# merlresearch/tssep

Hardware: AMD Instinct MI355X
Metric: frames/sec fwd+bwd, 4-spk TS-SEP, 16kHz 4s chunks (higher is better)
Workload: dtype bf16x3+f32

## Files before the change

tssep_amd/csrc/feat.hip:

```cpp
#include <math.h>
#include "common.h"

namespace {

__device__ __forceinline__ unsigned ord(float f) {
  const unsigned u = __float_as_uint(f);
  return (u & 0x80000000u) ? ~u : (u | 0x80000000u);
}
__device__ __forceinline__ float unord(unsigned u) {
  return __uint_as_float((u & 0x80000000u) ? (u & 0x7fffffffu) : ~u);
}

constexpr int MAXF = 1032;
constexpr int GSLOTS = 64;

struct FeatWs {
  unsigned* gmax;
  unsigned* umax;
  int* range;
  float* fbT;
  float* db;
};
constexpr int STAT_TF = 0, STAT_T = 1, STAT_F = 2;
__host__ __device__ inline int64_t feat_nmax(int64_t B, int F, int stat) { return stat == STAT_T ? B * F : B; }
__host__ __device__ inline FeatWs feat_ws(void* ws, int64_t B , int n_mels) {
  FeatWs w;
  char* p = (char*)ws;
  w.gmax = (unsigned*)p;
  w.umax = (unsigned*)(p + GSLOTS * 4);
  const int64_t off1 = GSLOTS * 4 + ((B * 4 + 15) / 16) * 16;
  w.range = (int*)(p + off1);
  const int64_t off2 = off1 + (((int64_t)2 * n_mels * 4 + 15) / 16) * 16;
  w.fbT = (float*)(p + off2);
  w.db = (float*)(p + off2 + (int64_t)n_mels * MAXF * 4);
  return w;
}

__global__ __launch_bounds__(64) void feat_init_kernel(void* ws, int64_t B, const float* __restrict__ fb,
                                                       int F, int n_mels) {
  FeatWs w = feat_ws(ws, B, n_mels);
  const int lane = threadIdx.x, m = blockIdx.x;
  if (m == 0) w.gmax[lane] = 0u;
  for (int64_t b = (int64_t)m * 64 + lane; b < B; b += (int64_t)gridDim.x * 64) w.umax[b] = 0u;
  if (m >= n_mels) return;
  float lo = (float)F, hi = 0.f;
  for (int f = lane; f < F; f += 64) {
    const float v = fb[(int64_t)f * n_mels + m];
    w.fbT[(int64_t)m * MAXF + f] = v;
    if (v != 0.f) { lo = fminf(lo, (float)f); hi = fmaxf(hi, (float)(f + 1)); }
  }
  lo = -wave_max(-lo);
  hi = wave_max(hi);
  if (lane == 0) {
    w.range[2 * m] = hi == 0.f ? 0 : (int)lo;
    w.range[2 * m + 1] = (int)hi;
  }
}

constexpr int FPW = 4;
constexpr int CWMAX = 2 * MAXF;
constexpr int LMELS = 128;

__global__ __launch_bounds__(256) void feat_pass1_kernel(const float2* __restrict__ X, int64_t B,
                                                         int64_t T, int F,
                                                         const float* __restrict__ fb, int n_mels,
                                                         int n_mfcc, void* ws, int stat, int log_mels) {
  __shared__ float pw[4][MAXF];
  __shared__ float cw[CWMAX];
  __shared__ int clo[LMELS], chi[LMELS], coff[LMELS + 1];
  __shared__ int s_packed;
  FeatWs w = feat_ws(ws, feat_nmax(B, F, stat), n_mels);
  const int tid = threadIdx.x, lane = tid & 63, wave = tid >> 6;
  if (n_mfcc > 0) {
    if (tid < n_mels && tid < LMELS) {
      clo[tid] = w.range[2 * tid];
      chi[tid] = w.range[2 * tid + 1];
    }
    __syncthreads();
    if (tid == 0) {
      int tot = 0;
      const int nm = n_mels < LMELS ? n_mels : LMELS;
      for (int m = 0; m < nm; ++m) {
        coff[m] = tot;
        const int wd = chi[m] - clo[m];
        tot += wd > 0 ? wd : 0;
      }
      coff[nm] = tot;
      s_packed = (n_mels <= LMELS && tot <= CWMAX) ? 1 : 0;
    }
    __syncthreads();
    if (s_packed)
      for (int m = wave; m < n_mels; m += 4)
        for (int f = clo[m] + lane; f < chi[m]; f += 64) cw[coff[m] + f - clo[m]] = w.fbT[(int64_t)m * MAXF + f];
    __syncthreads();
  }
  const bool packed = n_mfcc > 0 && s_packed;
  float dbmax = -INFINITY;
  for (int it = 0; it < FPW; ++it) {
    const int64_t frame = ((int64_t)blockIdx.x * FPW + it) * 4 + wave;
    if (frame >= B * T) break;
    const float2* x = X + frame * F;
    float amax = 0.f;
    float2 xv[17];
#pragma unroll
    for (int r = 0; r < 17; ++r) {
      const int f = lane + 64 * r;
      xv[r] = f < F ? x[f] : make_float2(0.f, 0.f);
    }
#pragma unroll
    for (int r = 0; r < 17; ++r) {
      const int f = lane + 64 * r;
      if (f < F) {
        const float p = xv[r].x * xv[r].x + xv[r].y * xv[r].y;
        pw[wave][f] = p;
        amax = fmaxf(amax, sqrtf(p));
        if (stat == STAT_T) {
          unsigned* slot = w.umax + (frame / T) * F + f;
          const unsigned o_ = ord(sqrtf(p));
          if (o_ > __hip_atomic_load(slot, __ATOMIC_RELAXED, __HIP_MEMORY_SCOPE_AGENT)) atomicMax(slot, o_);
        }
      }
    }
    __builtin_amdgcn_fence(__ATOMIC_RELEASE, "wavefront");
    __builtin_amdgcn_wave_barrier();
    __builtin_amdgcn_fence(__ATOMIC_ACQUIRE, "wavefront");
    amax = wave_max(amax);
    if (lane == 0 && stat == STAT_TF) atomicMax(w.umax + frame / T, ord(amax));
    if (n_mfcc > 0) {
      for (int m0 = 0; m0 < n_mels; m0 += 64) {
        float mine = 0.f;
        const int mm = n_mels - m0 < 64 ? n_mels - m0 : 64;
        if (lane < mm) {
          const int m = m0 + lane;
          const int lo = packed ? clo[m] : w.range[2 * m], hi = packed ? chi[m] : w.range[2 * m + 1];
          const float* frow = packed ? cw + coff[m] - lo : w.fbT + (int64_t)m * MAXF;
          const float* prow = pw[wave];
          float s0 = 0.f, s1 = 0.f, s2 = 0.f, s3 = 0.f;
          int f = lo;
          for (; f + 3 < hi; f += 4) {
            s0 = fmaf(prow[f], frow[f], s0);
            s1 = fmaf(prow[f + 1], frow[f + 1], s1);
            s2 = fmaf(prow[f + 2], frow[f + 2], s2);
            s3 = fmaf(prow[f + 3], frow[f + 3], s3);
          }
          if (f < hi) s0 = fmaf(prow[f], frow[f], s0);
          if (f + 1 < hi) s1 = fmaf(prow[f + 1], frow[f + 1], s1);
          if (f + 2 < hi) s2 = fmaf(prow[f + 2], frow[f + 2], s2);
          mine = (s0 + s1) + (s2 + s3);
        }
        if (lane < mm) {
          const float db = log_mels ? logf(mine + 1e-6f) : 10.0f * log10f(fmaxf(mine, 1e-10f));
          w.db[frame * n_mels + m0 + lane] = db;
          dbmax = fmaxf(dbmax, db);
        }
      }
    }
    __builtin_amdgcn_fence(__ATOMIC_RELEASE, "wavefront");
    __builtin_amdgcn_wave_barrier();
    __builtin_amdgcn_fence(__ATOMIC_ACQUIRE, "wavefront");
  }
  if (n_mfcc > 0) {
    dbmax = wave_max(dbmax);
    if (lane == 0 && dbmax > -INFINITY) atomicMax(w.gmax + (blockIdx.x & (GSLOTS - 1)), ord(dbmax));
  }
}

__global__ __launch_bounds__(256) void feat_pass2_kernel(const float2* __restrict__ X, int64_t B,
                                                         int64_t T, int F,
                                                         const float* __restrict__ dct, int n_mels,
                                                         int n_mfcc, float top_db,
                                                         float* __restrict__ out, int64_t ld_out,
                                                         const void* ws, int stat) {
  __shared__ float dbl[4][64];
  FeatWs w = feat_ws(const_cast<void*>(ws), feat_nmax(B, F, stat), n_mels);
  const int lane = threadIdx.x & 63, wave = threadIdx.x >> 6;
  const int64_t frame = (int64_t)blockIdx.x * 4 + wave;
  const bool valid = frame < B * T;
  float* o = out + (valid ? frame : 0) * ld_out;
  if (n_mfcc > 0) {
    const float floor_db = top_db < 0.f ? -INFINITY : wave_max(unord(w.gmax[lane])) - top_db;
    for (int m0 = 0; m0 < n_mels; m0 += 64) {
      if (valid && m0 + lane < n_mels)
        dbl[wave][lane] = fmaxf(w.db[frame * n_mels + m0 + lane], floor_db);
      __syncthreads();
      if (valid) {
        const int mm = n_mels - m0 < 64 ? n_mels - m0 : 64;
        for (int c = lane; c < n_mfcc; c += 64) {
          float s = m0 ? o[c] : 0.f;
          for (int m = 0; m < mm; ++m) s = fmaf(dbl[wave][m], dct[(int64_t)(m0 + m) * n_mfcc + c], s);
          o[c] = s;
        }
      }
      __syncthreads();
    }
  }
  if (!valid) return;
  const float2* x = X + frame * F;
  float2 xv[17];
#pragma unroll
  for (int r = 0; r < 17; ++r) {
    const int f = lane + 64 * r;
    xv[r] = f < F ? x[f] : make_float2(0.f, 0.f);
  }
  if (stat == STAT_TF) {
    const float scale = (float)(M_E - 1.0) / unord(w.umax[frame / T]);
#pragma unroll
    for (int r = 0; r < 17; ++r) {
      const int f = lane + 64 * r;
      if (f < F) o[n_mfcc + f] = log1pf(sqrtf(xv[r].x * xv[r].x + xv[r].y * xv[r].y) * scale);
    }
    return;
  }
  float fmx = 0.f;
  if (stat == STAT_F) {
#pragma unroll
    for (int r = 0; r < 17; ++r)
      if (lane + 64 * r < F) fmx = fmaxf(fmx, sqrtf(xv[r].x * xv[r].x + xv[r].y * xv[r].y));
    fmx = wave_max(fmx);
  }
#pragma unroll
  for (int r = 0; r < 17; ++r) {
    const int f = lane + 64 * r;
    if (f < F) {
      const float norm = stat == STAT_F ? fmx : unord(w.umax[(frame / T) * F + f]);
      o[n_mfcc + f] = log1pf(sqrtf(xv[r].x * xv[r].x + xv[r].y * xv[r].y) * ((float)(M_E - 1.0) / norm));
    }
  }
}

}

extern "C" int64_t tssep_feat_workspace_bytes(int64_t B, int64_t T, int n_mels, int F, int stat_axis) {
  if (stat_axis < 0 || stat_axis > 2 || F <= 0) return 0;
  FeatWs w = feat_ws(nullptr, feat_nmax(B, F, stat_axis), n_mels);
  return (int64_t)((char*)w.db - (char*)nullptr) + B * T * (int64_t)n_mels * 4 + 16;
}

extern "C" int tssep_feat_fwd(const float* X, int64_t B, int64_t T, int F, const float* fb,
                              const float* dct, int n_mels, int n_mfcc, float top_db, int stat_axis,
                              float* out, int64_t ld_out, void* ws, void* stream) {
  if (!X || !out || !ws) return TSSEP_E_NULL;
  if (n_mfcc > 0 && (!fb || !dct)) return TSSEP_E_NULL;
  if (B <= 0 || T <= 0 || F <= 0 || F > MAXF || ld_out < n_mfcc + F) return TSSEP_E_SHAPE;
  if (n_mfcc > 0 && (n_mels <= 0 || n_mels > 1024)) return TSSEP_E_SHAPE;
  if (n_mfcc == 0) n_mels = 0;
  if (stat_axis < 0 || stat_axis > 2) return TSSEP_E_SHAPE;
  if ((((uintptr_t)X) & 7u) || (((uintptr_t)ws) & 15u)) return TSSEP_E_ALIGN;
  hipStream_t s = (hipStream_t)stream;
  const int nm = n_mels > 0 ? n_mels : 1;
  const int64_t nmax = feat_nmax(B, F, stat_axis);
  const int64_t nb0 = (nmax + 64 * 16 - 1) / (64 * 16);
  hipLaunchKernelGGL(feat_init_kernel, dim3((unsigned)(nb0 > nm ? (nb0 > 4096 ? 4096 : nb0) : nm)), dim3(64), 0, s, ws, nmax, fb, F, n_mels);
  const unsigned blocks = (unsigned)((B * T + 3) / 4);
  const unsigned blocks1 = (unsigned)((B * T + 4 * FPW - 1) / (4 * FPW));
  hipLaunchKernelGGL(feat_pass1_kernel, dim3(blocks1), dim3(256), 0, s, (const float2*)X, B, T, F,
                     fb, n_mels, n_mfcc, ws, stat_axis, top_db < 0.f ? 1 : 0);
  hipLaunchKernelGGL(feat_pass2_kernel, dim3(blocks), dim3(256), 0, s, (const float2*)X, B, T, F,
                     dct, n_mels, n_mfcc, top_db, out, ld_out, ws, stat_axis);
  return tssep_launch_status();
}
```

Before: 2.159 million.

## Restructure feature kernels as persistent waves with prefetched buffer loads and LDS DCT

```diff
diff --git a/tssep_amd/csrc/feat.hip b/tssep_amd/csrc/feat.hip
--- a/tssep_amd/csrc/feat.hip
+++ b/tssep_amd/csrc/feat.hip
@@ -1,5 +1,6 @@
 #include <math.h>
 #include "common.h"
+#include "gemm_common.h"
 
 namespace {
 
@@ -57,107 +58,172 @@
   }
 }
 
-constexpr int FPW = 4;
-constexpr int CWMAX = 2 * MAXF;
+typedef __amdgpu_buffer_rsrc_t srd_t;
+typedef unsigned u32x4_t __attribute__((ext_vector_type(4)));
+__device__ __forceinline__ srd_t frame_srd(const float2* X, int64_t frame, int64_t nframes, int F) {
+  const bool in = frame < nframes;
+  return __builtin_amdgcn_make_buffer_rsrc(const_cast<float2*>(X + (in ? frame : 0) * F), 0, in ? F * 8 : 0, 0x00020000);
+}
+__device__ __forceinline__ f32x4 bload4(srd_t r, int voff) {
+  return __builtin_bit_cast(f32x4, __builtin_amdgcn_raw_buffer_load_b128(r, voff, 0, 0));
+}
+#define WAVE_SYNC()                                          \
+  do {                                                       \
+    __builtin_amdgcn_fence(__ATOMIC_RELEASE, "wavefront");   \
+    __builtin_amdgcn_wave_barrier();                         \
+    __builtin_amdgcn_fence(__ATOMIC_ACQUIRE, "wavefront");   \
+  } while (0)
+__device__ __forceinline__ float lane_value(float v, int l) {
+  return __int_as_float(__builtin_amdgcn_readlane(__float_as_int(v), l));
+}
+__device__ __forceinline__ float power(float re, float im) {
+#pragma clang fp contract(off)
+  return re * re + im * im;
+}
+
+constexpr int p1_occ(int NL) { return NL <= 5 ? 6 : 4; }
 constexpr int LMELS = 128;
-
-__global__ __launch_bounds__(256) void feat_pass1_kernel(const float2* __restrict__ X, int64_t B,
-                                                         int64_t T, int F,
-                                                         const float* __restrict__ fb, int n_mels,
-                                                         int n_mfcc, void* ws, int stat, int log_mels) {
-  __shared__ float pw[4][MAXF];
-  __shared__ float cw[CWMAX];
+constexpr int CWMAX = 2 * MAXF + 6 * LMELS;
+
+__host__ __device__ inline int seg_len(int lo, int hi) { return hi > lo ? ((hi + 3) & ~3) - (lo & ~3) : 0; }
+
+__device__ __forceinline__ float band_sum_global(const FeatWs& w, int m, const float* prow) {
+  const int lo = w.range[2 * m], hi = w.range[2 * m + 1];
+  const float* frow = w.fbT + (int64_t)m * MAXF;
+  float s0 = 0.f, s1 = 0.f, s2 = 0.f, s3 = 0.f;
+  int f = lo;
+  for (; f + 3 < hi; f += 4) {
+    s0 = fmaf(prow[f], frow[f], s0);
+    s1 = fmaf(prow[f + 1], frow[f + 1], s1);
+    s2 = fmaf(prow[f + 2], frow[f + 2], s2);
+    s3 = fmaf(prow[f + 3], frow[f + 3], s3);
+  }
+  if (f < hi) s0 = fmaf(prow[f], frow[f], s0);
+  if (f + 1 < hi) s1 = fmaf(prow[f + 1], frow[f + 1], s1);
+  if (f + 2 < hi) s2 = fmaf(prow[f + 2], frow[f + 2], s2);
+  return (s0 + s1) + (s2 + s3);
+}
+
+template <int NL>
+__global__ __launch_bounds__(256, p1_occ(NL)) void feat_pass1_kernel(const float2* __restrict__ X, int64_t B,
+                                                         int64_t T, int F, int n_mels,
+                                                         int n_mfcc, void* ws, int stat, int log_mels, int fpw) {
+  __shared__ __attribute__((aligned(16))) float pw[4][NL * 128];
+  __shared__ __attribute__((aligned(16))) float cw[CWMAX];
   __shared__ int clo[LMELS], chi[LMELS], coff[LMELS + 1];
   __shared__ int s_packed;
   FeatWs w = feat_ws(ws, feat_nmax(B, F, stat), n_mels);
-  const int tid = threadIdx.x, lane = tid & 63, wave = tid >> 6;
+  const int tid = threadIdx.x, lane = tid & 63;
+  const int wave = __builtin_amdgcn_readfirstlane(tid >> 6);
   if (n_mfcc > 0) {
-    if (tid < n_mels && tid < LMELS) {
+    const int nm = n_mels < LMELS ? n_mels : LMELS;
+    if (tid < nm) {
       clo[tid] = w.range[2 * tid];
       chi[tid] = w.range[2 * tid + 1];
     }
     __syncthreads();
-    if (tid == 0) {
-      int tot = 0;
-      const int nm = n_mels < LMELS ? n_mels : LMELS;
-      for (int m = 0; m < nm; ++m) {
-        coff[m] = tot;
-        const int wd = chi[m] - clo[m];
-        tot += wd > 0 ? wd : 0;
-      }
-      coff[nm] = tot;
-      s_packed = (n_mels <= LMELS && tot <= CWMAX) ? 1 : 0;
+    if (tid < nm) {
+      int off = 0, len = 0;
+#pragma unroll 8
+      for (int j = 0; j < nm; ++j) {
+        const int l = seg_len(clo[j], chi[j]);
+        off += j < tid ? l : 0;
+        len = j == tid ? l : len;
+      }
+      coff[tid] = off;
+      if (tid == nm - 1) {
+        coff[nm] = off + len;
+        s_packed = (n_mels <= LMELS && off + len <= CWMAX) ? 1 : 0;
+      }
     }
     __syncthreads();
     if (s_packed)
-      for (int m = wave; m < n_mels; m += 4)
-        for (int f = clo[m] + lane; f < chi[m]; f += 64) cw[coff[m] + f - clo[m]] = w.fbT[(int64_t)m * MAXF + f];
+      for (int m = wave; m < n_mels; m += 4) {
+        const int lo = clo[m], hi = chi[m], a = lo & ~3, n = seg_len(lo, hi);
+        for (int j = lane; j < n; j += 64) {
+          const int f = a + j;
+          cw[coff[m] + j] = (f >= lo && f < hi) ? w.fbT[(int64_t)m * MAXF + f] : 0.f;
+        }
+      }
     __syncthreads();
   }
   const bool packed = n_mfcc > 0 && s_packed;
+  const int64_t nfr = B * T;
+  const int64_t f0 = ((int64_t)blockIdx.x * 4 + wave) * fpw;
+  if (f0 >= nfr) return;
+  const int64_t f1 = nfr - f0 < fpw ? nfr : f0 + fpw;
+  int64_t utt = f0 / T, utt_end = (utt + 1) * T;
+  float* prow = pw[wave];
+  const int voff = lane * 16;
+  f32x4 cur[NL], nxt[NL];
+  {
+    const srd_t r0 = frame_srd(X, f0, f1, F);
+#pragma unroll
+    for (int r = 0; r < NL; ++r) cur[r] = bload4(r0, voff + 1024 * r);
+  }
+  int lo_r = 0, nq_r = 0, wo_r = 0;
+  if (packed && lane < n_mels) {
+    lo_r = clo[lane];
+    nq_r = seg_len(lo_r, chi[lane]) >> 2;
+    wo_r = coff[lane];
+  }
   float dbmax = -INFINITY;
-  for (int it = 0; it < FPW; ++it) {
-    const int64_t frame = ((int64_t)blockIdx.x * FPW + it) * 4 + wave;
-    if (frame >= B * T) break;
-    const float2* x = X + frame * F;
-    float amax = 0.f;
-    float2 xv[17];
-#pragma unroll
-    for (int r = 0; r < 17; ++r) {
-      const int f = lane + 64 * r;
-      xv[r] = f < F ? x[f] : make_float2(0.f, 0.f);
-    }
-#pragma unroll
-    for (int r = 0; r < 17; ++r) {
-      const int f = lane + 64 * r;
-      if (f < F) {
-        const float p = xv[r].x * xv[r].x + xv[r].y * xv[r].y;
-        pw[wave][f] = p;
-        amax = fmaxf(amax, sqrtf(p));
-        if (stat == STAT_T) {
-          unsigned* slot = w.umax + (frame / T) * F + f;
-          const unsigned o_ = ord(sqrtf(p));
-          if (o_ > __hip_atomic_load(slot, __ATOMIC_RELAXED, __HIP_MEMORY_SCOPE_AGENT)) atomicMax(slot, o_);
-        }
-      }
-    }
-    __builtin_amdgcn_fence(__ATOMIC_RELEASE, "wavefront");
-    __builtin_amdgcn_wave_barrier();
-    __builtin_amdgcn_fence(__ATOMIC_ACQUIRE, "wavefront");
-    amax = wave_max(amax);
-    if (lane == 0 && stat == STAT_TF) atomicMax(w.umax + frame / T, ord(amax));
+#pragma unroll 1
+  for (int64_t frame = f0; frame < f1; ++frame) {
+    {
+      const srd_t r1 = frame_srd(X, frame + 1, f1, F);
+#pragma unroll
+      for (int r = 0; r < NL; ++r) nxt[r] = bload4(r1, voff + 1024 * r);
+    }
+    float pmax = 0.f;
+#pragma unroll
+    for (int r = 0; r < NL; ++r) {
+      const int f = 128 * r + 2 * lane;
+      const float p0 = power(cur[r].x, cur[r].y), p1 = power(cur[r].z, cur[r].w);
+      *reinterpret_cast<float2*>(prow + f) = make_float2(p0, p1);
+      pmax = fmaxf(pmax, fmaxf(p0, p1));
+      if (stat == STAT_T) {
+        unsigned* slot = w.umax + utt * F + f;
+        const unsigned o0 = ord(p0), o1 = ord(p1);
+        if (f < F && o0 > __hip_atomic_load(slot, __ATOMIC_RELAXED, __HIP_MEMORY_SCOPE_AGENT)) atomicMax(slot, o0);
+        if (f + 1 < F && o1 > __hip_atomic_load(slot + 1, __ATOMIC_RELAXED, __HIP_MEMORY_SCOPE_AGENT)) atomicMax(slot + 1, o1);
+      }
+    }
+    WAVE_SYNC();
+    pmax = wave_max(pmax);
+    if (lane == 0 && stat == STAT_TF) atomicMax(w.umax + utt, ord(sqrtf(pmax)));
     if (n_mfcc > 0) {
       for (int m0 = 0; m0 < n_mels; m0 += 64) {
-        float mine = 0.f;
-        const int mm = n_mels - m0 < 64 ? n_mels - m0 : 64;
-        if (lane < mm) {
-          const int m = m0 + lane;
-          const int lo = packed ? clo[m] : w.range[2 * m], hi = packed ? chi[m] : w.range[2 * m + 1];
-          const float* frow = packed ? cw + coff[m] - lo : w.fbT + (int64_t)m * MAXF;
-          const float* prow = pw[wave];
-          float s0 = 0.f, s1 = 0.f, s2 = 0.f, s3 = 0.f;
-          int f = lo;
-          for (; f + 3 < hi; f += 4) {
-            s0 = fmaf(prow[f], frow[f], s0);
-            s1 = fmaf(prow[f + 1], frow[f + 1], s1);
-            s2 = fmaf(prow[f + 2], frow[f + 2], s2);
-            s3 = fmaf(prow[f + 3], frow[f + 3], s3);
+        const int m = m0 + lane;
+        if (m < n_mels) {
+          float mine;
+          if (packed) {
+            const int lo = m0 ? clo[m] : lo_r;
+            const int nq = m0 ? seg_len(lo, chi[m]) >> 2 : nq_r;
+            const f32x4* pq = reinterpret_cast<const f32x4*>(prow + (lo & ~3));
+            const f32x4* wq = reinterpret_cast<const f32x4*>(cw + (m0 ? coff[m] : wo_r));
+            float t0 = 0.f, t1 = 0.f, t2 = 0.f, t3 = 0.f;
+            for (int q = 0; q < nq; ++q) {
+              const f32x4 p = pq[q], c = wq[q];
+              t0 = fmaf(p.x, c.x, t0);
+              t1 = fmaf(p.y, c.y, t1);
+              t2 = fmaf(p.z, c.z, t2);
+              t3 = fmaf(p.w, c.w, t3);
+            }
+            mine = (lo & 1) ? (t1 + t2) + (t0 + t3) : (t0 + t1) + (t2 + t3);
+          } else {
+            mine = band_sum_global(w, m, prow);
           }
-          if (f < hi) s0 = fmaf(prow[f], frow[f], s0);
-          if (f + 1 < hi) s1 = fmaf(prow[f + 1], frow[f + 1], s1);
-          if (f + 2 < hi) s2 = fmaf(prow[f + 2], frow[f + 2], s2);
-          mine = (s0 + s1) + (s2 + s3);
-        }
-        if (lane < mm) {
           const float db = log_mels ? logf(mine + 1e-6f) : 10.0f * log10f(fmaxf(mine, 1e-10f));
-          w.db[frame * n_mels + m0 + lane] = db;
+          w.db[frame * n_mels + m] = db;
           dbmax = fmaxf(dbmax, db);
         }
       }
     }
-    __builtin_amdgcn_fence(__ATOMIC_RELEASE, "wavefront");
-    __builtin_amdgcn_wave_barrier();
-    __builtin_amdgcn_fence(__ATOMIC_ACQUIRE, "wavefront");
+    WAVE_SYNC();
+    if (frame + 1 >= utt_end) { ++utt; utt_end += T; }
+#pragma unroll
+    for (int r = 0; r < NL; ++r) cur[r] = nxt[r];
   }
   if (n_mfcc > 0) {
     dbmax = wave_max(dbmax);
@@ -165,65 +231,136 @@
   }
 }
 
-__global__ __launch_bounds__(256) void feat_pass2_kernel(const float2* __restrict__ X, int64_t B,
+constexpr int P2_OCC = 6;
+constexpr int G2 = 32;
+constexpr int DLMAX = 6144;
+
+__device__ __forceinline__ void pass2_frame_generic(const float2* __restrict__ x, int F, int lane, int stat,
+                                                    const unsigned* umax_row, float* __restrict__ o) {
+  float2 xv[17];
+#pragma unroll
+  for (int r = 0; r < 17; ++r) {
+    const int f = lane + 64 * r;
+    xv[r] = f < F ? x[f] : make_float2(0.f, 0.f);
+  }
+  float fmx = 0.f;
+  if (stat == STAT_F) {
+#pragma unroll
+    for (int r = 0; r < 17; ++r)
+      if (lane + 64 * r < F) fmx = fmaxf(fmx, power(xv[r].x, xv[r].y));
+    fmx = sqrtf(wave_max(fmx));
+  }
+#pragma unroll
+  for (int r = 0; r < 17; ++r) {
+    const int f = lane + 64 * r;
+    if (f < F) {
+      const float norm = stat == STAT_F ? fmx : sqrtf(unord(umax_row[f]));
+      o[f] = log1pf(sqrtf(power(xv[r].x, xv[r].y)) * ((float)(M_E - 1.0) / norm));
+    }
+  }
+}
+
+template <int NL, bool TF>
+__global__ __launch_bounds__(256, P2_OCC) void feat_pass2_kernel(const float2* __restrict__ X, int64_t B,
                                                          int64_t T, int F,
                                                          const float* __restrict__ dct, int n_mels,
                                                          int n_mfcc, float top_db,
                                                          float* __restrict__ out, int64_t ld_out,
-                                                         const void* ws, int stat) {
+                                                         const void* ws, int stat, int fpw) {
+  __shared__ float dl[DLMAX];
   __shared__ float dbl[4][64];
+  __shared__ float scl[4][G2];
+  static_assert((160 * 1024) / (int)(sizeof(dl) + sizeof(dbl) + sizeof(scl)) == P2_OCC, "LDS admits P2_OCC workgroups per CU");
   FeatWs w = feat_ws(const_cast<void*>(ws), feat_nmax(B, F, stat), n_mels);
-  const int lane = threadIdx.x & 63, wave = threadIdx.x >> 6;
-  const int64_t frame = (int64_t)blockIdx.x * 4 + wave;
-  const bool valid = frame < B * T;
-  float* o = out + (valid ? frame : 0) * ld_out;
-  if (n_mfcc > 0) {
-    const float floor_db = top_db < 0.f ? -INFINITY : wave_max(unord(w.gmax[lane])) - top_db;
-    for (int m0 = 0; m0 < n_mels; m0 += 64) {
-      if (valid && m0 + lane < n_mels)
-        dbl[wave][lane] = fmaxf(w.db[frame * n_mels + m0 + lane], floor_db);
-      __syncthreads();
-      if (valid) {
-        const int mm = n_mels - m0 < 64 ? n_mels - m0 : 64;
-        for (int c = lane; c < n_mfcc; c += 64) {
-          float s = m0 ? o[c] : 0.f;
-          for (int m = 0; m < mm; ++m) s = fmaf(dbl[wave][m], dct[(int64_t)(m0 + m) * n_mfcc + c], s);
-          o[c] = s;
+  const int tid = threadIdx.x, lane = tid & 63;
+  const int wave = __builtin_amdgcn_readfirstlane(tid >> 6);
+  const bool dct_lds = n_mfcc > 0 && n_mels <= 64 && n_mels * n_mfcc <= DLMAX;
+  if (dct_lds) {
+    for (int i = tid; i < n_mels * n_mfcc; i += 256) dl[i] = dct[i];
+    __syncthreads();
+  }
+  const int64_t nfr = B * T;
+  const int64_t f0 = ((int64_t)blockIdx.x * 4 + wave) * fpw;
+  if (f0 >= nfr) return;
+  const int64_t f1 = nfr - f0 < fpw ? nfr : f0 + fpw;
+  const float floor_db = n_mfcc <= 0 || top_db < 0.f ? -INFINITY : wave_max(unord(w.gmax[lane])) - top_db;
+  const int np = F >> 7, Fb = np << 7, R = F - Fb;
+  const bool st8 = ((((uintptr_t)out) | ((uintptr_t)ld_out * 4) | ((uintptr_t)n_mfcc * 4)) & 7u) == 0;
+  const int voff = lane * 16;
+  int64_t utt = f0 / T, utt_end = (utt + 1) * T;
+  for (int64_t g0 = f0; g0 < f1; g0 += G2) {
+    const int ng = f1 - g0 < G2 ? (int)(f1 - g0) : G2;
+#pragma unroll 1
+    for (int j = 0; j < ng; ++j) {
+      const int64_t frame = g0 + j;
+      float* o = out + frame * ld_out;
+      f32x4 x4[NL];
+      if (TF) {
+        const srd_t r0 = frame_srd(X, frame, f1, F);
+#pragma unroll
+        for (int r = 0; r < NL; ++r) x4[r] = bload4(r0, voff + 1024 * r);
+      }
+      if (n_mfcc > 0) {
+        if (dct_lds) {
+          const float dbv = lane < n_mels ? fmaxf(w.db[frame * n_mels + lane], floor_db) : 0.f;
+          for (int c0 = 0; c0 < n_mfcc; c0 += 64) {
+            const int c = c0 + lane < n_mfcc ? c0 + lane : n_mfcc - 1;
+            const float* dc = dl + c;
+            float s = 0.f;
+            int m = 0;
+            for (; m + 4 <= n_mels; m += 4) {
+              const float d0 = dc[m * n_mfcc], d1 = dc[(m + 1) * n_mfcc], d2 = dc[(m + 2) * n_mfcc], d3 = dc[(m + 3) * n_mfcc];
+              s = fmaf(lane_value(dbv, m), d0, s);
+              s = fmaf(lane_value(dbv, m + 1), d1, s);
+              s = fmaf(lane_value(dbv, m + 2), d2, s);
+              s = fmaf(lane_value(dbv, m + 3), d3, s);
+            }
+            for (; m < n_mels; ++m) s = fmaf(lane_value(dbv, m), dc[m * n_mfcc], s);
+            if (c0 + lane < n_mfcc) o[c] = s;
+          }
+        } else {
+          for (int m0 = 0; m0 < n_mels; m0 += 64) {
+            if (m0 + lane < n_mels) dbl[wave][lane] = fmaxf(w.db[frame * n_mels + m0 + lane], floor_db);
+            WAVE_SYNC();
+            const int mm = n_mels - m0 < 64 ? n_mels - m0 : 64;
+            for (int c = lane; c < n_mfcc; c += 64) {
+              float s = m0 ? o[c] : 0.f;
+              for (int m = 0; m < mm; ++m) s = fmaf(dbl[wave][m], dct[(int64_t)(m0 + m) * n_mfcc + c], s);
+              o[c] = s;
+            }
+            WAVE_SYNC();
+          }
         }
       }
-      __syncthreads();
-    }
-  }
-  if (!valid) return;
-  const float2* x = X + frame * F;
-  float2 xv[17];
-#pragma unroll
-  for (int r = 0; r < 17; ++r) {
-    const int f = lane + 64 * r;
-    xv[r] = f < F ? x[f] : make_float2(0.f, 0.f);
-  }
-  if (stat == STAT_TF) {
-    const float scale = (float)(M_E - 1.0) / unord(w.umax[frame / T]);
-#pragma unroll
-    for (int r = 0; r < 17; ++r) {
-      const int f = lane + 64 * r;
-      if (f < F) o[n_mfcc + f] = log1pf(sqrtf(xv[r].x * xv[r].x + xv[r].y * xv[r].y) * scale);
-    }
-    return;
-  }
-  float fmx = 0.f;
-  if (stat == STAT_F) {
-#pragma unroll
-    for (int r = 0; r < 17; ++r)
-      if (lane + 64 * r < F) fmx = fmaxf(fmx, sqrtf(xv[r].x * xv[r].x + xv[r].y * xv[r].y));
-    fmx = wave_max(fmx);
-  }
-#pragma unroll
-  for (int r = 0; r < 17; ++r) {
-    const int f = lane + 64 * r;
-    if (f < F) {
-      const float norm = stat == STAT_F ? fmx : unord(w.umax[(frame / T) * F + f]);
-      o[n_mfcc + f] = log1pf(sqrtf(xv[r].x * xv[r].x + xv[r].y * xv[r].y) * ((float)(M_E - 1.0) / norm));
+      while (frame >= utt_end) { ++utt; utt_end += T; }
+      if (!TF) {
+        pass2_frame_generic(X + frame * F, F, lane, stat, w.umax + utt * F, o + n_mfcc);
+        continue;
+      }
+      const float scale = (float)(M_E - 1.0) / unord(w.umax[utt]);
+      if (lane == 0) scl[wave][j] = scale;
+      o += n_mfcc + 2 * lane;
+#pragma unroll
+      for (int r = 0; r < NL; ++r)
+        if (r < np) {
+          const float y0 = log1pf(sqrtf(power(x4[r].x, x4[r].y)) * scale);
+          const float y1 = log1pf(sqrtf(power(x4[r].z, x4[r].w)) * scale);
+          if (st8) {
+            *reinterpret_cast<float2*>(o + 128 * r) = make_float2(y0, y1);
+          } else {
+            o[128 * r] = y0;
+            o[128 * r + 1] = y1;
+          }
+        }
+    }
+    if (TF && R > 0) {
+      WAVE_SYNC();
+      for (int idx = lane; idx < ng * R; idx += 64) {
+        const int j = idx / R, f = Fb + idx - j * R;
+        const float2 xv = X[(g0 + j) * F + f];
+        out[(g0 + j) * ld_out + n_mfcc + f] = log1pf(sqrtf(power(xv.x, xv.y)) * scl[wave][j]);
+      }
+      WAVE_SYNC();
     }
   }
 }
@@ -251,11 +388,22 @@
   const int64_t nmax = feat_nmax(B, F, stat_axis);
   const int64_t nb0 = (nmax + 64 * 16 - 1) / (64 * 16);
   hipLaunchKernelGGL(feat_init_kernel, dim3((unsigned)(nb0 > nm ? (nb0 > 4096 ? 4096 : nb0) : nm)), dim3(64), 0, s, ws, nmax, fb, F, n_mels);
-  const unsigned blocks = (unsigned)((B * T + 3) / 4);
-  const unsigned blocks1 = (unsigned)((B * T + 4 * FPW - 1) / (4 * FPW));
-  hipLaunchKernelGGL(feat_pass1_kernel, dim3(blocks1), dim3(256), 0, s, (const float2*)X, B, T, F,
-                     fb, n_mels, n_mfcc, ws, stat_axis, top_db < 0.f ? 1 : 0);
-  hipLaunchKernelGGL(feat_pass2_kernel, dim3(blocks), dim3(256), 0, s, (const float2*)X, B, T, F,
-                     dct, n_mels, n_mfcc, top_db, out, ld_out, ws, stat_axis);
+  const int64_t nfr = B * T, cus = gemm_detail::current_device_cus();
+  const int nl1 = F + 3 <= 5 * 128 ? 5 : 9;
+  const int64_t nb1 = (nfr + 3) / 4 < cus * p1_occ(nl1) ? (nfr + 3) / 4 : cus * p1_occ(nl1);
+  const int64_t nb2 = (nfr + 3) / 4 < cus * P2_OCC ? (nfr + 3) / 4 : cus * P2_OCC;
+  const int64_t fpw1 = (nfr + nb1 * 4 - 1) / (nb1 * 4), fpw2 = (nfr + nb2 * 4 - 1) / (nb2 * 4);
+  if (fpw1 > 0x7fffffff) return TSSEP_E_SHAPE;
+  const float2* Xc = (const float2*)X;
+  const int lm = top_db < 0.f ? 1 : 0;
+  if (nl1 == 5)
+    hipLaunchKernelGGL(feat_pass1_kernel<5>, dim3((unsigned)nb1), dim3(256), 0, s, Xc, B, T, F, n_mels, n_mfcc, ws, stat_axis, lm,
+                       (int)fpw1);
+  else
+    hipLaunchKernelGGL(feat_pass1_kernel<9>, dim3((unsigned)nb1), dim3(256), 0, s, Xc, B, T, F, n_mels, n_mfcc, ws, stat_axis, lm,
+                       (int)fpw1);
+  auto pass2 = stat_axis != STAT_TF ? feat_pass2_kernel<4, false> : (F >> 7) <= 4 ? feat_pass2_kernel<4, true> : feat_pass2_kernel<8, true>;
+  hipLaunchKernelGGL(pass2, dim3((unsigned)nb2), dim3(256), 0, s, Xc, B, T, F, dct, n_mels, n_mfcc, top_db, out, ld_out, ws,
+                     stat_axis, (int)fpw2);
   return tssep_launch_status();
 }
```

Result: no change. 2.159 million (-0.0%).
